# ArseneAmoya/image-retrieval-wavelet

Measured on AMD Instinct MI355X. Metric: query images/sec + mAP@5000, MIRFLICKR-25k 64-bit hash, 1/2/4/8 MI355X, higher is better.
Workload: dtype f32; 1 GPU; c1: MIRFLICKR-25k shape, retrieval-only: per GPU per step 2048 query images 3x224x224 u8 -> SWT db2 L3 -> band-attention head (Nq=4, E=384; DINOv2 backbone out of scope, CLS features synthetic) -> 64-bit hash -> Hamming top-5000 vs 25,000 codes -> mAP@5000; queries_per_gpu=2048, db_codes=25000, nbits=64, k=5000, wavelet=db2, level=3, arithmetic=fp32 SWT and head (fp32 MFMA), 64-bit popcount ranking, AP in fp32/fp64, streams=1, clock_steps=40, backend=none, parallelism=single GPU

## Files before the change

image-retrieval-wavelet_amd/csrc/ap_walk.hpp:

```cpp
#pragma once
#include "common.hpp"

namespace wv {

constexpr int kApRounds = 32;

template <int TPQ>
__host__ __device__ constexpr int ap_scratch_dwords() { return kApRounds * (TPQ / 64) + 2 * (TPQ / 64) + 2; }

struct ApState {
    uint32_t running = 0;
    double acc = 0.0;
};

template <int TPQ>
__device__ __forceinline__ void ap_accum(uint32_t relbits, const uint32_t *cnt, int Rc, int r_base, int t, ApState &st)
{
    constexpr int NW = TPQ / 64, CH = 8;
    const int wv = t >> 6;
    for (int r0 = 0; r0 < Rc; r0 += CH) {
        uint32_t c[CH][NW];
#pragma unroll
        for (int u = 0; u < CH; ++u)
#pragma unroll
            for (int w2 = 0; w2 < NW; ++w2) c[u][w2] = cnt[min(r0 + u, Rc - 1) * NW + w2];
#pragma unroll
        for (int u = 0; u < CH; ++u) {
            const int r = r0 + u;
            if (r < Rc) {
                uint32_t before = st.running, tot = 0;
#pragma unroll
                for (int w2 = 0; w2 < NW; ++w2) {
                    before += w2 < wv ? c[u][w2] : 0u;
                    tot += c[u][w2];
                }
                const bool rel = (relbits >> r) & 1u;
                const uint64_t m = __ballot(rel);
                if (rel) {
                    const uint32_t j = before + (uint32_t)mbcnt(m) + 1;
                    st.acc += (double)((float)j / (float)((r_base + r) * TPQ + t + 1));
                }
                st.running += tot;
            }
        }
    }
}

template <int TPQ, typename SYNC>
__device__ __forceinline__ void ap_final(const ApState &st, double *wsum, int t, float *__restrict__ ap_out,
                                         int32_t *__restrict__ nrel_out, SYNC group_barrier)
{
    constexpr int NW = TPQ / 64;
    const int lane = t & 63, wv = t >> 6;
    const double acc = wave_sum_f64(st.acc);
    if (lane == 0) wsum[wv] = acc;
    group_barrier();
    if (t == 0) {
        double s = wsum[0];
#pragma unroll
        for (int w2 = 1; w2 < NW; ++w2) s += wsum[w2];
        *ap_out = st.running ? (float)(s / (double)st.running) : 0.0f;
        if (nrel_out) *nrel_out = (int32_t)st.running;
    }
}

constexpr int kMaxCutoffs = 16;

struct ApCuts {
    int n;
    int k[kMaxCutoffs];
};

template <int TPQ>
__host__ __device__ constexpr int ap_cuts_scratch_dwords() { return ap_scratch_dwords<TPQ>() + TPQ / 64; }

template <int TPQ, typename SYNC>
__device__ __forceinline__ void ap_accum_cuts(uint32_t relbits, const uint32_t *cnt, int Rc, int r_base, int t, ApState &st,
                                              const ApCuts &cuts, int &next, double *wsum, uint32_t *wcut,
                                              float *__restrict__ ap_out, int32_t *__restrict__ nrel_out, SYNC group_barrier)
{
    constexpr int NW = TPQ / 64, CH = 8;
    const int lane = t & 63, wv = t >> 6;
    int64_t cut = next < cuts.n ? cuts.k[next] : INT64_MAX;
    for (int r0 = 0; r0 < Rc; r0 += CH) {
        uint32_t c[CH][NW];
#pragma unroll
        for (int u = 0; u < CH; ++u)
#pragma unroll
            for (int w2 = 0; w2 < NW; ++w2) c[u][w2] = cnt[min(r0 + u, Rc - 1) * NW + w2];
#pragma unroll
        for (int u = 0; u < CH; ++u) {
            const int r = r0 + u;
            if (r < Rc) {
                uint32_t before = st.running, tot = 0;
#pragma unroll
                for (int w2 = 0; w2 < NW; ++w2) {
                    before += w2 < wv ? c[u][w2] : 0u;
                    tot += c[u][w2];
                }
                const bool rel = (relbits >> r) & 1u;
                const uint64_t m = __ballot(rel);
                const int p = (r_base + r) * TPQ + t;
                double own = 0.0;
                if (rel) {
                    const uint32_t j = before + (uint32_t)mbcnt(m) + 1;
                    own = (double)((float)j / (float)(p + 1));
                }
                while (cut <= (int64_t)(r_base + r + 1) * TPQ) {
                    const bool in = rel && p < cut;
                    const uint64_t mc = __ballot(in);
                    const double acc = wave_sum_f64(in ? st.acc + own : st.acc);
                    if (lane == 0) {
                        wsum[wv] = acc;
                        wcut[wv] = (uint32_t)__popcll(mc);
                    }
                    group_barrier();
                    if (t == 0) {
                        double s = wsum[0];
                        uint32_t running = st.running + wcut[0];
#pragma unroll
                        for (int w2 = 1; w2 < NW; ++w2) {
                            s += wsum[w2];
                            running += wcut[w2];
                        }
                        ap_out[next] = running ? (float)(s / (double)running) : 0.0f;
                        if (nrel_out) nrel_out[next] = (int32_t)running;
                    }
                    group_barrier();
                    ++next;
                    cut = next < cuts.n ? cuts.k[next] : INT64_MAX;
                }
                if (rel) st.acc += own;
                st.running += tot;
            }
        }
    }
}

}
```

image-retrieval-wavelet_amd/csrc/rank.hpp:

```cpp
#pragma once
#include "common.hpp"

namespace wv {

struct ApCuts;

constexpr int kTopkThreads = 256;
constexpr int kMaxBins = 130;
constexpr int kWinBins = 32;
constexpr int kWinRows = kWinBins + 1;
constexpr size_t kRankLdsLimit = 100 * 1024;

enum class RankKernel {
    none,
    column,
    window256,
    window64,
};

enum class RankMode {
    lists,
    rows16,
    hist,
    ap,
    relbits,
    radius,
};

constexpr int64_t kImg64MaxRows = 64 * 64;
constexpr int64_t kImg256MaxRows = 256 * 128;

constexpr int rank_threads_per_query(RankKernel kern) { return kern == RankKernel::window64 ? 64 : 256; }

struct RankPlan {
    RankKernel kernel;
    int C;
    int NC;
    size_t lds;
    const char *why;
    const char *instead;
};

__host__ __device__ inline int rank2_bitmap_words(int64_t N) { return (int)((N + 31) / 32); }

inline size_t window_lds_bytes_per_query(int tpq, int k, int bm_words = 0)
{
    size_t b = (size_t)kWinRows * (tpq / 2) * 4;
    b += ((size_t)(k + tpq) * 2 + 15) / 16 * 16;
    b += (size_t)(kMaxBins + 1 + kWinBins + 4 + 3) / 4 * 4 * 4;
    b += (size_t)bm_words * 4;
    b = (b + 15) / 16 * 16;
    const size_t hist = (size_t)(kMaxBins + 1) * 17 * 4;
    return b > hist ? b : (hist + 15) / 16 * 16;
}

constexpr int rank_radius_bitmap_words(int C) { return 8 * C + 1; }
inline size_t radius_lds_bytes(int C)
{
    const size_t b = (size_t)(kMaxBins + 1) * 16 * 4 + (size_t)2 * (kMaxBins + 1) * 4 + (size_t)rank_radius_bitmap_words(C) * 4;
    return (b + 15) / 16 * 16;
}

inline bool column_u16(int64_t n_items) { return n_items < 65536; }
inline size_t column_lds_bytes(int nbins, bool u16)
{
    const size_t h = (size_t)nbins * (u16 ? kTopkThreads / 2 : kTopkThreads);
    return (h + kMaxBins + kMaxBins + 1 + 4 + 3) / 4 * 4 * sizeof(uint32_t);
}

inline RankPlan rank_plan_column(int64_t N, int nbits)
{
    return {RankKernel::column, (int)ceil_div(N, kTopkThreads), 0, column_lds_bytes(nbits + 1, column_u16(N)), nullptr, ""};
}

inline RankKernel rank_window_kernel(int Q, int64_t N, int k)
{
    const char *force = ::wv::tune("WV_TOPK_V2");
    if (force && force[0] == '0') return RankKernel::none;
    if (N >= 65536 || 2 * (k + 128) >= 65536) return RankKernel::none;
    const bool fits256 = N <= kImg256MaxRows && window_lds_bytes_per_query(256, k) <= kRankLdsLimit;
    const bool fits64 = N <= kImg64MaxRows && 4 * window_lds_bytes_per_query(64, k) <= kRankLdsLimit;
    if (force && atoi(force) == 64 && fits64) return RankKernel::window64;
    if (force && atoi(force) == 256 && fits256) return RankKernel::window256;
    if (fits64 && Q >= 4096) return RankKernel::window64;
    return fits256 ? RankKernel::window256 : (fits64 ? RankKernel::window64 : RankKernel::none);
}

inline RankPlan rank_plan(int Q, int64_t N, int nbits, int k, RankMode mode)
{
    const bool fused = mode == RankMode::ap || mode == RankMode::relbits;
    const char *instead = mode == RankMode::ap ? "; call wv_hamming_topk + wv_map_at_k instead" : "";
    RankKernel kern = rank_window_kernel(Q, N, std::max(k, 1));
    if (kern == RankKernel::none) {
        if (mode == RankMode::lists) return rank_plan_column(N, nbits);
        return {RankKernel::none, 0, 0, 0, "are outside the windowed kernel (rows <= 32768, 16-bit row numbers: 2 (k + 128) < 65536)",
                instead};
    }
    if (fused && kern == RankKernel::window64 && k > 32 * 64) kern = RankKernel::window256;
    if (mode == RankMode::radius) kern = RankKernel::window256;
    RankPlan p{kern, 0, 0, 0, nullptr, ""};
    const int tpq = rank_threads_per_query(kern);
    p.C = (int)ceil_div(N, tpq);
    p.NC = p.C <= 16 ? 4 : (p.C <= 32 ? 8 : (p.C <= 64 ? 16 : (p.C <= 100 ? 25 : 32)));
    p.lds = window_lds_bytes_per_query(tpq, k, fused ? rank2_bitmap_words(N) : 0) * (kTopkThreads / tpq);
    if (mode == RankMode::radius) p.lds = radius_lds_bytes(p.C);
    if (fused && p.lds > kRankLdsLimit)
        return {RankKernel::none, 0, 0, 0, "do not fit the fused kernel's LDS (list + relevance bitmap)", instead};
    return p;
}

inline int rank_refuse(const char *what, const RankPlan &p, int64_t N, int k)
{
    WV_FAIL(WV_ENOTSUP, "%s: %lld rows / k=%d %s%s", what, (long long)N, k, p.why, p.instead);
}

inline size_t rank_image_bytes(RankKernel kern, int64_t N, int words)
{
    if (kern == RankKernel::column) return (size_t)ceil_div(N, kTopkThreads) * kTopkThreads * words * sizeof(uint64_t);
    const int tpq = rank_threads_per_query(kern);
    const int64_t C = ceil_div(N, tpq), rows = words == 1 ? (C + 1) / 2 : C;
    return (size_t)rows * tpq * 16;
}

struct BlobLayout {
    size_t column, window256, window64, total;
};
inline BlobLayout blob_layout(int64_t N, int words)
{
    BlobLayout L;
    L.column = L.window256 = L.window64 = L.total = (size_t)align_up((int64_t)dist_prepared_bytes(N, words), 256);
    if (words > 2) return L;
    L.window256 = L.column + (size_t)align_up((int64_t)rank_image_bytes(RankKernel::column, N, words), 256);
    L.window64 = L.window256 + (N <= kImg256MaxRows ? (size_t)align_up((int64_t)rank_image_bytes(RankKernel::window256, N, words), 256) : 0);
    L.total = L.window64 + (N <= kImg64MaxRows ? rank_image_bytes(RankKernel::window64, N, words) : 0);
    return L;
}
inline const void *blob_image(const void *prepared, int64_t N, int words, RankKernel kern)
{
    const BlobLayout L = blob_layout(N, words);
    return (const char *)prepared + (kern == RankKernel::column ? L.column : (kern == RankKernel::window256 ? L.window256 : L.window64));
}

int rank2_prepare(const uint64_t *db, void *img, int64_t N, int words, RankKernel kern, hipStream_t st);
size_t rank2_labels_bytes(int64_t N, int lwords);
int rank2_labels_prepare(const uint64_t *dblab, void *cls, int64_t N, int lwords, hipStream_t st);

struct Rank2Ap {
    const uint32_t *cls;
    const uint64_t *qlab;
    int lwords;
    float *ap;
    int32_t *nrel;
    uint64_t *relbits;
    int64_t relbits_ld;
    int64_t cum_ld;
};

int rank2_launch(const RankPlan &plan, const uint64_t *q, const void *img, int32_t *idx, uint16_t *rows16, uint8_t *dist,
                 uint32_t *cum, int Q, int64_t N, int nbits, int k, int64_t idx_offset, hipStream_t st,
                 const Rank2Ap *apx = nullptr, const ApCuts *cuts = nullptr);

int rank2_radius_launch(const RankPlan &plan, const uint64_t *q, const void *img, const Rank2Ap &apx, uint32_t *cum, uint32_t *cumrel,
                        int Q, int64_t N, int nbits, hipStream_t st);

}
```

image-retrieval-wavelet_amd/csrc/rank2.hip:

```cpp
#include "rank.hpp"
#include "ap_walk.hpp"

namespace wv {

#ifdef WV_RANK2_STAMPS
__device__ unsigned long long g_rank2_stamps[8];
#define R2_STAMP(i) do { __builtin_amdgcn_sched_barrier(0); const unsigned long long now_ = __builtin_amdgcn_s_memtime(); \
    __builtin_amdgcn_s_waitcnt(0xC07F); if (t == 0) atomicAdd(&g_rank2_stamps[i], now_ - stamp_); stamp_ = __builtin_amdgcn_s_memtime(); \
    __builtin_amdgcn_sched_barrier(0); } while (0)
#define R2_STAMP_INIT unsigned long long stamp_ = __builtin_amdgcn_s_memtime()
#else
#define R2_STAMP(i) do { } while (0)
#define R2_STAMP_INIT do { } while (0)
#endif

template <int WORDS>
struct QCode {
    uint64_t w[WORDS];
};

template <int TPQ>
__device__ __forceinline__ void group_sync()
{
    if constexpr (TPQ == 64) {
// ... 552 lines not shown

template <int WORDS, int TPQ, int NC, bool AP>
__global__ __launch_bounds__(256, rank2_min_waves(NC)) void k_rank_window(const uint64_t *__restrict__ q, const uint4 *__restrict__ img,
                                                     int32_t *__restrict__ idx, uint16_t *__restrict__ rows16,
                                                     uint8_t *__restrict__ dist, int Q, int64_t N, int C, int nbins, int k,
                                                     int64_t idx_offset, uint32_t *__restrict__ cum, int lds_per_group, Rank2Ap apx)
{
    extern __shared__ uint4 lds4[];
    constexpr int GPW = 256 / TPQ;
    const int g = threadIdx.x / TPQ, t = threadIdx.x % TPQ;
    const int qi = blockIdx.x * GPW + g;
    if (qi >= Q) return;
    uint8_t *lds = reinterpret_cast<uint8_t *>(lds4) + (size_t)g * lds_per_group;
    QCode<WORDS> qc;
#pragma unroll
    for (int w = 0; w < WORDS; ++w) {
        const uint64_t v = q[(int64_t)qi * WORDS + w];
        qc.w[w] = ((uint64_t)(uint32_t)__builtin_amdgcn_readfirstlane((int)(uint32_t)(v >> 32)) << 32) |
                  (uint32_t)__builtin_amdgcn_readfirstlane((int)(uint32_t)v);
    }
    if (k != 0) rank2_zero_table<TPQ>(lds, t);
    uint32_t dc[NC], dmin;
    rank2_distances<WORDS, TPQ, NC>(img, qc, N, C, t, dc, dmin);
#pragma unroll
    for (int once = 0; once < 1; ++once) {
        if (k == 0) {
            rank2_hist_only<TPQ, NC>(dc, N, C, nbins, cum + (int64_t)qi * (nbins + 1), lds, t);
            continue;
        }
        group_sync<TPQ>();
        if constexpr (AP) {
            const uint64_t lw = apx.qlab[(int64_t)qi * apx.lwords], lw2 = apx.lwords > 1 ? apx.qlab[(int64_t)qi * apx.lwords + 1] : 0;
            const uint64_t ql = ((uint64_t)(uint32_t)__builtin_amdgcn_readfirstlane((int)(uint32_t)(lw >> 32)) << 32) |
                                (uint32_t)__builtin_amdgcn_readfirstlane((int)(uint32_t)lw);
            const uint64_t ql2 = ((uint64_t)(uint32_t)__builtin_amdgcn_readfirstlane((int)(uint32_t)(lw2 >> 32)) << 32) |
                                 (uint32_t)__builtin_amdgcn_readfirstlane((int)(uint32_t)lw2);
            rank2_rank<TPQ, NC, 1>(dc, dmin, N, C, nbins, k,
                                      cum ? cum + (int64_t)qi * (apx.cum_ld ? apx.cum_ld : nbins + 1) : nullptr, nullptr, lds, t,
                                      apx.cls, ql, ql2, apx.ap ? apx.ap + qi : nullptr, apx.nrel ? apx.nrel + qi : nullptr,
                                      apx.relbits ? apx.relbits + (int64_t)qi * (apx.relbits_ld ? apx.relbits_ld : (k + 63) / 64)
                                                  : nullptr);
        } else {
            rank2_rank<TPQ, NC>(dc, dmin, N, C, nbins, k, cum ? cum + (int64_t)qi * (nbins + 1) : nullptr,
                                dist ? dist + (int64_t)qi * k : nullptr, lds, t);
            rank2_copy_list<TPQ>(lds, k, idx_offset, idx ? idx + (int64_t)qi * k : nullptr,
                                 rows16 ? rows16 + (int64_t)qi * k : nullptr, t);
        }
    }
}

constexpr int rank2_cuts_min_waves(int nc) { return nc <= 8 ? 6 : rank2_min_waves(nc); }

template <int WORDS, int TPQ, int NC>
__global__ __launch_bounds__(256, rank2_cuts_min_waves(NC)) void k_rank_window_cuts(const uint64_t *__restrict__ q, const uint4 *__restrict__ img,
                                                                               int Q, int64_t N, int C, int nbins, int lds_per_group,
                                                                               Rank2Ap apx, ApCuts cuts)
{
    extern __shared__ uint4 lds4[];
    constexpr int GPW = 256 / TPQ;
    const int g = threadIdx.x / TPQ, t = threadIdx.x % TPQ;
    const int qi = blockIdx.x * GPW + g;
    if (qi >= Q) return;
    uint8_t *lds = reinterpret_cast<uint8_t *>(lds4) + (size_t)g * lds_per_group;
    QCode<WORDS> qc;
#pragma unroll
    for (int w = 0; w < WORDS; ++w) {
        const uint64_t v = q[(int64_t)qi * WORDS + w];
        qc.w[w] = ((uint64_t)(uint32_t)__builtin_amdgcn_readfirstlane((int)(uint32_t)(v >> 32)) << 32) |
                  (uint32_t)__builtin_amdgcn_readfirstlane((int)(uint32_t)v);
    }
    rank2_zero_table<TPQ>(lds, t);
    uint32_t dc[NC], dmin;
    rank2_distances<WORDS, TPQ, NC>(img, qc, N, C, t, dc, dmin);
    group_sync<TPQ>();
    const uint64_t lw = apx.qlab[(int64_t)qi * apx.lwords], lw2 = apx.lwords > 1 ? apx.qlab[(int64_t)qi * apx.lwords + 1] : 0;
    const uint64_t ql = ((uint64_t)(uint32_t)__builtin_amdgcn_readfirstlane((int)(uint32_t)(lw >> 32)) << 32) |
                        (uint32_t)__builtin_amdgcn_readfirstlane((int)(uint32_t)lw);
    const uint64_t ql2 = ((uint64_t)(uint32_t)__builtin_amdgcn_readfirstlane((int)(uint32_t)(lw2 >> 32)) << 32) |
                         (uint32_t)__builtin_amdgcn_readfirstlane((int)(uint32_t)lw2);
    rank2_rank<TPQ, NC, 2>(dc, dmin, N, C, nbins, cuts.k[cuts.n - 1], nullptr, nullptr, lds, t, apx.cls, ql, ql2,
                           apx.ap + (int64_t)qi * cuts.n, apx.nrel ? apx.nrel + (int64_t)qi * cuts.n : nullptr, nullptr, &cuts);
}

template <int TPQ, int NC>
__device__ __forceinline__ void rank2_radius_hist(const uint32_t (&dc)[NC], int C, int nbins, const uint32_t *bitmap, uint32_t *table,
                                                  uint32_t *tot, uint32_t *__restrict__ cum_out, uint32_t *__restrict__ cumrel_out, int t)
{
    const int first = t * C;
    char *cell = reinterpret_cast<char *>(table) + (uint32_t)(t & 15) * 4u;
#pragma unroll
    for (int bw = 0; bw < NC; bw += 8) {
        if (bw * 4 < C) {
            const int p = first + bw * 4;
            const uint32_t lo = bitmap[p >> 5], hi = bitmap[(p >> 5) + 1];
            const uint32_t rel32 = (uint32_t)((((uint64_t)hi << 32) | lo) >> (p & 31));
#pragma unroll
            for (int j = 0; j < 32; ++j) {
                if (bw + (j >> 2) < NC) {
                    const uint32_t d = (dc[bw + (j >> 2)] >> (8 * (j & 3))) & 0xffu;
                    const uint32_t b = min(d, (uint32_t)nbins);
                    const uint32_t inc = 1u + (((rel32 >> j) & 1u) << 16);
                    __hip_atomic_fetch_add(reinterpret_cast<uint32_t *>(cell + b * 64), inc, __ATOMIC_RELAXED,
                                           __HIP_MEMORY_SCOPE_WORKGROUP);
                }
            }
            __builtin_amdgcn_sched_barrier(0);
        }
    }
    group_sync<TPQ>();
    for (int b = t; b < nbins; b += TPQ) {
        const uint4 *row = reinterpret_cast<const uint4 *>(table + b * 16);
        uint32_t all = 0, rel = 0;
#pragma unroll
        for (int i = 0; i < 4; ++i) {
            const uint4 v = row[i];
            all += (v.x & 0xffffu) + (v.y & 0xffffu) + (v.z & 0xffffu) + (v.w & 0xffffu);
            rel += (v.x >> 16) + (v.y >> 16) + (v.z >> 16) + (v.w >> 16);
        }
        tot[b] = all;
        tot[kMaxBins + 1 + b] = rel;
    }
    group_sync<TPQ>();
    if (t < 128) {
        const int which = __builtin_amdgcn_readfirstlane(t >> 6), b0 = 3 * (t & 63);
        const uint32_t *src = tot + which * (kMaxBins + 1);
        uint32_t *dst = which ? cumrel_out : cum_out;
        const uint32_t t0 = b0 < nbins ? src[b0] : 0u, t1 = b0 + 1 < nbins ? src[b0 + 1] : 0u, t2 = b0 + 2 < nbins ? src[b0 + 2] : 0u;
        const uint32_t incl = wave_incl_scan_u32(t0 + t1 + t2), excl = incl - (t0 + t1 + t2);
        if (b0 <= nbins) dst[b0] = excl;
        if (b0 + 1 <= nbins) dst[b0 + 1] = excl + t0;
        if (b0 + 2 <= nbins) dst[b0 + 2] = excl + t0 + t1;
    }
}

template <int WORDS, int TPQ, int NC>
__global__ __launch_bounds__(256, rank2_min_waves(NC)) void k_rank_radius(const uint64_t *__restrict__ q, const uint4 *__restrict__ img,
                                                                          int Q, int64_t N, int C, int nbins, Rank2Ap apx,
                                                                          uint32_t *__restrict__ cum, uint32_t *__restrict__ cumrel)
{
    static_assert(TPQ == 256, "the radius histograms are built for 256 threads per query (rank_plan never picks another)");
    extern __shared__ uint4 lds4[];
    const int t = threadIdx.x;
    const int qi = blockIdx.x;
    if (qi >= Q) return;
    uint32_t *table = reinterpret_cast<uint32_t *>(lds4);
    uint32_t *tot = table + (kMaxBins + 1) * 16;
    uint32_t *bitmap = tot + 2 * (kMaxBins + 1);
    QCode<WORDS> qc;
#pragma unroll
    for (int w = 0; w < WORDS; ++w) {
        const uint64_t v = q[(int64_t)qi * WORDS + w];
        qc.w[w] = ((uint64_t)(uint32_t)__builtin_amdgcn_readfirstlane((int)(uint32_t)(v >> 32)) << 32) |
                  (uint32_t)__builtin_amdgcn_readfirstlane((int)(uint32_t)v);
    }
    const int nw = rank2_bitmap_words(N);
    for (int i = t; i < (nbins + 1) * 16; i += TPQ) table[i] = 0;
    for (int w = nw + t; w < rank_radius_bitmap_words(C); w += TPQ) bitmap[w] = 0;
    uint32_t dc[NC], dmin;
    rank2_distances<WORDS, TPQ, NC>(img, qc, N, C, t, dc, dmin);
    (void)dmin;
    const uint64_t lw = apx.qlab[(int64_t)qi * apx.lwords], lw2 = apx.lwords > 1 ? apx.qlab[(int64_t)qi * apx.lwords + 1] : 0;
    const uint64_t ql = ((uint64_t)(uint32_t)__builtin_amdgcn_readfirstlane((int)(uint32_t)(lw >> 32)) << 32) |
                        (uint32_t)__builtin_amdgcn_readfirstlane((int)(uint32_t)lw);
    const uint64_t ql2 = ((uint64_t)(uint32_t)__builtin_amdgcn_readfirstlane((int)(uint32_t)(lw2 >> 32)) << 32) |
                         (uint32_t)__builtin_amdgcn_readfirstlane((int)(uint32_t)lw2);
    rank2_relevance_bitmap<TPQ>(apx.cls, ql, ql2, nw, t, bitmap);
    group_sync<TPQ>();
    rank2_radius_hist<TPQ, NC>(dc, C, nbins, bitmap, table, tot, cum + (int64_t)qi * (nbins + 1), cumrel + (int64_t)qi * (nbins + 1), t);
}

int rank2_prepare(const uint64_t *db, void *img, int64_t N, int words, RankKernel kern, hipStream_t st)
{
    const int tpq = rank_threads_per_query(kern);
    const int C = (int)ceil_div(N, tpq);
    const int64_t total = (int64_t)(words == 1 ? (C + 1) / 2 : C) * tpq;
    const unsigned grid = (unsigned)std::min<int64_t>(ceil_div(total, 256), 4096);
    if (words == 1)
        hipLaunchKernelGGL((k_rank2_image<1>), dim3(grid), dim3(256), 0, st, db, (uint4 *)img, N, C, tpq);
    else
        hipLaunchKernelGGL((k_rank2_image<2>), dim3(grid), dim3(256), 0, st, db, (uint4 *)img, N, C, tpq);
    WV_CHECK_LAUNCH("k_rank2_image");
    return WV_OK;
}

namespace {
struct WindowArgs {
    const uint64_t *q;
    const void *img;
    int32_t *idx;
    uint16_t *rows16;
    uint8_t *dist;
    uint32_t *cum;
    int Q;
    int64_t N;
    int nbins, k;
    int64_t idx_offset;
    hipStream_t st;
    bool fused;
    Rank2Ap apx;
    const ApCuts *cuts;
};

template <int WORDS, int TPQ, int NC>
int launch_window(const RankPlan &plan, const WindowArgs &a)
{
    constexpr int GPW = 256 / TPQ;
    if (a.cuts) {
        auto kc = k_rank_window_cuts<WORDS, TPQ, NC>;
        if (plan.lds > 64 * 1024) {
            hipError_t e = hipFuncSetAttribute(reinterpret_cast<const void *>(kc), hipFuncAttributeMaxDynamicSharedMemorySize, (int)plan.lds);
            if (e != hipSuccess) WV_FAIL(WV_EHIP, "rank_window_cuts: hipFuncSetAttribute(%zu): %s", plan.lds, hipGetErrorString(e));
        }
        hipLaunchKernelGGL(kc, dim3((unsigned)ceil_div(a.Q, GPW)), dim3(256), plan.lds, a.st, a.q, (const uint4 *)a.img, a.Q, a.N, plan.C,
                           a.nbins, (int)(plan.lds / GPW), a.apx, *a.cuts);
        WV_CHECK_LAUNCH("k_rank_window_cuts");
        return WV_OK;
    }
    auto kern = a.fused ? k_rank_window<WORDS, TPQ, NC, true> : k_rank_window<WORDS, TPQ, NC, false>;
    if (plan.lds > 64 * 1024) {
        hipError_t e = hipFuncSetAttribute(reinterpret_cast<const void *>(kern), hipFuncAttributeMaxDynamicSharedMemorySize, (int)plan.lds);
        if (e != hipSuccess) WV_FAIL(WV_EHIP, "rank_window: hipFuncSetAttribute(%zu): %s", plan.lds, hipGetErrorString(e));
    }
    hipLaunchKernelGGL(kern, dim3((unsigned)ceil_div(a.Q, GPW)), dim3(256), plan.lds, a.st, a.q, (const uint4 *)a.img, a.idx, a.rows16,
                       a.dist, a.Q, a.N, plan.C, a.nbins, a.k, a.idx_offset, a.cum, (int)(plan.lds / GPW), a.apx);
    WV_CHECK_LAUNCH("k_rank_window");
    return WV_OK;
}

template <int WORDS, int TPQ>
int launch_window_nc(const RankPlan &plan, const WindowArgs &a)
{
    if (plan.NC == 4) return launch_window<WORDS, TPQ, 4>(plan, a);
    if (plan.NC == 8) return launch_window<WORDS, TPQ, 8>(plan, a);
    if constexpr (TPQ == 256) {
        if (plan.NC == 25) return launch_window<WORDS, TPQ, 25>(plan, a);
        if (plan.NC == 32) return launch_window<WORDS, TPQ, 32>(plan, a);
    }
    return launch_window<WORDS, TPQ, 16>(plan, a);
}
}

int rank2_launch(const RankPlan &plan, const uint64_t *q, const void *img, int32_t *idx, uint16_t *rows16, uint8_t *dist,
                 uint32_t *cum, int Q, int64_t N, int nbits, int k, int64_t idx_offset, hipStream_t st, const Rank2Ap *apx,
                 const ApCuts *cuts)
{
    const WindowArgs a{q, img, idx, rows16, dist, cum, Q, N, nbits + 1, k, idx_offset, st, apx != nullptr, apx ? *apx : Rank2Ap{}, cuts};
    const bool wave = plan.kernel == RankKernel::window64;
    if (nbits <= 64) return wave ? launch_window_nc<1, 64>(plan, a) : launch_window_nc<1, 256>(plan, a);
    return wave ? launch_window_nc<2, 64>(plan, a) : launch_window_nc<2, 256>(plan, a);
}

namespace {
template <int WORDS, int NC>
int launch_radius(const RankPlan &plan, const uint64_t *q, const void *img, const Rank2Ap &apx, uint32_t *cum, uint32_t *cumrel, int Q,
                  int64_t N, int nbins, hipStream_t st)
{
    hipLaunchKernelGGL((k_rank_radius<WORDS, 256, NC>), dim3((unsigned)Q), dim3(256), plan.lds, st, q, (const uint4 *)img, Q, N, plan.C,
                       nbins, apx, cum, cumrel);
    WV_CHECK_LAUNCH("k_rank_radius");
    return WV_OK;
}

template <int WORDS>
int launch_radius_nc(const RankPlan &plan, const uint64_t *q, const void *img, const Rank2Ap &apx, uint32_t *cum, uint32_t *cumrel, int Q,
                     int64_t N, int nbins, hipStream_t st)
{
    if (plan.NC == 4) return launch_radius<WORDS, 4>(plan, q, img, apx, cum, cumrel, Q, N, nbins, st);
    if (plan.NC == 8) return launch_radius<WORDS, 8>(plan, q, img, apx, cum, cumrel, Q, N, nbins, st);
    if (plan.NC == 16) return launch_radius<WORDS, 16>(plan, q, img, apx, cum, cumrel, Q, N, nbins, st);
    if (plan.NC == 25) return launch_radius<WORDS, 25>(plan, q, img, apx, cum, cumrel, Q, N, nbins, st);
    return launch_radius<WORDS, 32>(plan, q, img, apx, cum, cumrel, Q, N, nbins, st);
}
}

int rank2_radius_launch(const RankPlan &plan, const uint64_t *q, const void *img, const Rank2Ap &apx, uint32_t *cum, uint32_t *cumrel,
                        int Q, int64_t N, int nbits, hipStream_t st)
{
    if (plan.kernel != RankKernel::window256) WV_FAIL(WV_EINVAL, "rank2_radius_launch: the plan names no 256-thread kernel");
    if (nbits <= 64) return launch_radius_nc<1>(plan, q, img, apx, cum, cumrel, Q, N, nbits + 1, st);
    return launch_radius_nc<2>(plan, q, img, apx, cum, cumrel, Q, N, nbits + 1, st);
}

}

#ifdef WV_RANK2_STAMPS
extern "C" int wv_debug_rank2_stamps(unsigned long long *host8)
{
    if (hipMemcpyFromSymbol(host8, HIP_SYMBOL(wv::g_rank2_stamps), 8 * sizeof(unsigned long long)) != hipSuccess) return -5;
    unsigned long long zero[8] = {0, 0, 0, 0, 0, 0, 0, 0};
    if (hipMemcpyToSymbol(HIP_SYMBOL(wv::g_rank2_stamps), zero, sizeof(zero)) != hipSuccess) return -5;
    return 0;
}
#endif
```

image-retrieval-wavelet_amd/csrc/topk.hip:

```cpp
#include "rank.hpp"
#include "ap_walk.hpp"

namespace wv {

template <int WORDS>
struct CodeSource {
    const uint64_t *dbT;
    uint64_t qw[WORDS];
    int64_t idx_offset;
    struct Raw {
        uint64_t w[WORDS];
    };
    __device__ __forceinline__ Raw fetch(int r, int t, int64_t) const
    {
        const uint64_t *p = dbT + ((int64_t)r * kTopkThreads + t) * WORDS;
        Raw c;
        if constexpr (WORDS == 2) {
            const uint4 v = *reinterpret_cast<const uint4 *>(p);
            c.w[0] = (uint64_t)v.x | ((uint64_t)v.y << 32);
            c.w[1] = (uint64_t)v.z | ((uint64_t)v.w << 32);
        } else {
#pragma unroll
            for (int w = 0; w < WORDS; ++w) c.w[w] = p[w];
        }
// ... 992 lines not shown
        if (int rc = require_workspace(what, workspace, workspace_bytes, Q, N, nbits, k)) return rc;
    hipStream_t st = (hipStream_t)stream;
    const void *img = nullptr;
    if (int rc = rank_image(plan, db, prepared, workspace, N, (nbits + 63) / 64, st, &img)) return rc;
    return rank2_launch(plan, q, img, nullptr, rows16, nullptr, cum, Q, N, nbits, k, 0, st);
}

extern "C" int wv_hamming_hist(const uint64_t *q, const uint64_t *db, const void *prepared, uint32_t *cum, int Q, int64_t N,
                               int nbits, void *workspace, size_t workspace_bytes, void *stream)
{
    if (int rc = validate_rank_shape("hamming_hist", q && cum && (db || prepared), Q, N, nbits)) return rc;
    if (Q == 0) return WV_OK;
    return shard_call("hamming_hist", RankMode::hist, q, db, prepared, nullptr, cum, Q, N, nbits, 0, workspace, workspace_bytes, stream);
}

extern "C" int wv_hamming_shard_prefix(const uint64_t *q, const uint64_t *db, const void *prepared, uint16_t *rows, uint32_t *cum,
                                       int Q, int64_t N, int nbits, int k, void *workspace, size_t workspace_bytes, void *stream)
{
    if (int rc = validate_rank_args("hamming_shard_prefix", q && rows && cum && (db || prepared), Q, N, nbits, k)) return rc;
    if (Q == 0) return WV_OK;
    return shard_call("hamming_shard_prefix", RankMode::rows16, q, db, prepared, rows, cum, Q, N, nbits, k, workspace, workspace_bytes,
                      stream);
}

extern "C" int wv_hamming_shard_relbits(const uint64_t *q, const void *prepared, const void *prepared_labels, const uint64_t *qlab,
                                        int lwords, uint64_t *relbits, int64_t relbits_ld, uint32_t *cum, int64_t cum_ld, int Q,
                                        int64_t N, int nbits, int k, void *stream)
{
    WV_REQUIRE(lwords >= 1, "hamming_shard_relbits: lwords=%d", lwords);
    if (lwords > 2) WV_FAIL(WV_ENOTSUP, "hamming_shard_relbits: %d label words (more than 128 classes)", lwords);
    WV_REQUIRE((relbits_ld == 0 || relbits_ld >= (k + 63) / 64) && (cum_ld == 0 || cum_ld >= nbits + 2),
               "hamming_shard_relbits: row pitches %lld / %lld too small", (long long)relbits_ld, (long long)cum_ld);
    if (int rc = validate_rank_args("hamming_shard_relbits", q && prepared && prepared_labels && qlab && relbits && cum, Q, N, nbits, k))
        return rc;
    if (Q == 0) return WV_OK;
    const Rank2Ap apx{(const uint32_t *)prepared_labels, qlab, lwords, nullptr, nullptr, relbits, relbits_ld, cum_ld};
    return fused_call("hamming_shard_relbits", RankMode::relbits, q, prepared, apx, cum, Q, N, nbits, k, stream);
}

extern "C" int wv_merge_relbits_map(const uint64_t *relbits, int64_t relbits_ld, const uint32_t *cum, int64_t cum_ld, int G, int Q,
                                    int kin, int k, int nbits, float *ap, int32_t *nrel, int32_t *need_out, void *stream)
{
    WV_REQUIRE((relbits_ld == 0 || relbits_ld >= (kin + 63) / 64) && (cum_ld == 0 || cum_ld >= nbits + 2),
               "merge_relbits_map: row pitches %lld / %lld too small", (long long)relbits_ld, (long long)cum_ld);
    WV_REQUIRE(relbits && cum && ap, "merge_relbits_map: null buffer");
    WV_REQUIRE(G >= 1 && Q >= 0 && kin >= 1 && k >= 1, "merge_relbits_map: bad shape G=%d Q=%d kin=%d k=%d", G, Q, kin, k);
    if (int rc = require_nbits("merge_relbits_map", nbits)) return rc;
    if (Q == 0) return WV_OK;
    const int nbins = nbits + 1, w32 = 2 * (int)ceil_div(kin, 64), mwords = (k + 31) / 32 + 1;
    const size_t lds = ((size_t)G * (nbins + 1) + nbins + 1 + mwords + (mwords & 1) + ap_scratch_dwords<256>() + 4) * 4;
    WV_REQUIRE(lds <= 60 * 1024, "merge_relbits_map: too many shards (G=%d)", G);
    hipLaunchKernelGGL(k_merge_relbits_ap, dim3(Q), dim3(256), lds, (hipStream_t)stream, reinterpret_cast<const uint32_t *>(relbits),
                       cum, G, Q, kin, w32, k, nbins, ap, nrel, need_out, relbits_ld ? 2 * relbits_ld : (int64_t)w32,
                       cum_ld ? cum_ld : (int64_t)(nbins + 1));
    WV_CHECK_LAUNCH("k_merge_relbits_ap");
    return WV_OK;
}

static int validate_cuts(const char *what, const int *ks, int nk, int64_t limit, const char *limit_name, ApCuts &cuts)
{
    static_assert(kMaxCutoffs == WV_MAX_CUTOFFS, "ap_walk.hpp and wvhash.h disagree");
    WV_REQUIRE(ks, "%s: null cut-off list", what);
    WV_REQUIRE(nk >= 1 && nk <= kMaxCutoffs, "%s: %d cut-offs (supported: 1..%d)", what, nk, kMaxCutoffs);
    cuts.n = nk;
    for (int i = 0; i < kMaxCutoffs; ++i) cuts.k[i] = i < nk ? ks[i] : 0;
    WV_REQUIRE(ks[0] >= 1, "%s: cut-off %d must be >= 1", what, ks[0]);
    for (int i = 1; i < nk; ++i)
        WV_REQUIRE(ks[i] > ks[i - 1], "%s: cut-offs must be strictly ascending (ks[%d]=%d after %d)", what, i, ks[i], ks[i - 1]);
    WV_REQUIRE(ks[nk - 1] <= limit, "%s: largest cut-off %d must be <= %s=%lld", what, ks[nk - 1], limit_name, (long long)limit);
    return WV_OK;
}

extern "C" int wv_hamming_map_at_ks(const uint64_t *q, const void *prepared, const void *prepared_labels, const uint64_t *qlab,
                                    int lwords, int Q, int64_t N, int nbits, const int *ks, int nk, float *ap, int32_t *nrel,
                                    void *stream)
{
    WV_REQUIRE(lwords >= 1, "hamming_map_at_ks: lwords=%d", lwords);
    if (lwords > 2) WV_FAIL(WV_ENOTSUP, "hamming_map_at_ks: %d label words (more than 128 classes): wv_hamming_topk + wv_map_at_ks", lwords);
    if (int rc = validate_rank_shape("hamming_map_at_ks", q && prepared && prepared_labels && qlab && ap, Q, N, nbits)) return rc;
    ApCuts cuts;
    if (int rc = validate_cuts("hamming_map_at_ks", ks, nk, N, "N", cuts)) return rc;
    if (Q == 0) return WV_OK;
    const int kmax = cuts.k[nk - 1];
    const RankPlan plan = rank_plan(Q, N, nbits, kmax, RankMode::ap);
    if (plan.kernel == RankKernel::none)
        WV_FAIL(WV_ENOTSUP, "hamming_map_at_ks: %lld rows / largest cut-off %d %s; call wv_hamming_topk + wv_map_at_ks instead",
                (long long)N, kmax, plan.why);
    const Rank2Ap apx{(const uint32_t *)prepared_labels, qlab, lwords, ap, nrel, nullptr, 0, 0};
    return rank2_launch(plan, q, blob_image(prepared, N, (nbits + 63) / 64, plan.kernel), nullptr, nullptr, nullptr, nullptr, Q, N, nbits,
                        kmax, 0, (hipStream_t)stream, &apx, &cuts);
}

extern "C" size_t wv_merge_relbits_map_ks_lds_bytes(int G, int kmax, int nbits)
{
    if (G < 1 || kmax < 1 || nbits < 1 || nbits > 128) return 0;
    const int nbins = nbits + 1;
    const size_t mwords = (size_t)(kmax + 31) / 32 + 1;
    return ((size_t)G * (nbins + 1) + nbins + 1 + ap_cuts_scratch_dwords<256>() + 4) * 4 + (mwords + (mwords & 1)) * 4;
}

extern "C" int wv_merge_relbits_map_ks(const uint64_t *relbits, int64_t relbits_ld, const uint32_t *cum, int64_t cum_ld, int G, int Q,
                                       int kin, const int *ks, int nk, int nbits, float *ap, int32_t *nrel, int32_t *need_out,
                                       void *stream)
{
    WV_REQUIRE((relbits_ld == 0 || relbits_ld >= (kin + 63) / 64) && (cum_ld == 0 || cum_ld >= nbits + 2),
               "merge_relbits_map_ks: row pitches %lld / %lld too small", (long long)relbits_ld, (long long)cum_ld);
    WV_REQUIRE(relbits && cum && ap, "merge_relbits_map_ks: null buffer");
    WV_REQUIRE(G >= 1 && Q >= 0 && kin >= 1, "merge_relbits_map_ks: bad shape G=%d Q=%d kin=%d", G, Q, kin);
    if (int rc = require_nbits("merge_relbits_map_ks", nbits)) return rc;
    ApCuts cuts;
    if (int rc = validate_cuts("merge_relbits_map_ks", ks, nk, 0x7fffffff, "INT_MAX", cuts)) return rc;
    if (Q == 0) return WV_OK;
    const int kmax = cuts.k[nk - 1], nbins = nbits + 1, w32 = 2 * (int)ceil_div(kin, 64);
    const size_t lds = wv_merge_relbits_map_ks_lds_bytes(G, kmax, nbits), limit = WV_MERGE_RELBITS_LDS_LIMIT;
    if (lds > limit)
        WV_FAIL(WV_ENOTSUP, "merge_relbits_map_ks: the merged string of the largest cut-off %d does not fit LDS beside the run boundaries "
                "of G=%d shards (%zu bytes needed, %zu available)", kmax, G, lds, limit);
    hipLaunchKernelGGL(k_merge_relbits_ap_cuts, dim3(Q), dim3(256), lds, (hipStream_t)stream, reinterpret_cast<const uint32_t *>(relbits),
                       cum, G, Q, kin, w32, nbins, ap, nrel, need_out, relbits_ld ? 2 * relbits_ld : (int64_t)w32,
                       cum_ld ? cum_ld : (int64_t)(nbins + 1), cuts);
    WV_CHECK_LAUNCH("k_merge_relbits_ap_cuts");
    return WV_OK;
}

extern "C" int wv_map_at_ks(const int32_t *idx, int64_t ld, int Q, const int *ks, int nk, const uint64_t *qlab, const uint64_t *dblab,
                            int lwords, float *ap, int32_t *nrel, void *stream)
{
    WV_REQUIRE(idx && qlab && dblab && ap, "map_at_ks: null buffer");
    WV_REQUIRE(Q >= 0 && lwords >= 1 && ld >= 1, "map_at_ks: bad shape Q=%d ld=%lld lwords=%d", Q, (long long)ld, lwords);
    ApCuts cuts;
    if (int rc = validate_cuts("map_at_ks", ks, nk, ld, "ld", cuts)) return rc;
    if (Q == 0) return WV_OK;
    hipStream_t st = (hipStream_t)stream;
    if (lwords == 1)
        hipLaunchKernelGGL((k_map_at_ks<1>), dim3(Q), dim3(256), 0, st, idx, ld, qlab, dblab, lwords, ap, nrel, cuts);
    else if (lwords == 2)
        hipLaunchKernelGGL((k_map_at_ks<2>), dim3(Q), dim3(256), 0, st, idx, ld, qlab, dblab, lwords, ap, nrel, cuts);
    else
        hipLaunchKernelGGL((k_map_at_ks<0>), dim3(Q), dim3(256), 0, st, idx, ld, qlab, dblab, lwords, ap, nrel, cuts);
    WV_CHECK_LAUNCH("k_map_at_ks");
    return WV_OK;
}

extern "C" int wv_hamming_topk_rows16(const uint64_t *q, const uint64_t *db, const void *prepared, uint16_t *rows, int Q,
                                      int64_t N, int nbits, int k, void *workspace, size_t workspace_bytes, void *stream)
{
    if (int rc = validate_rank_args("hamming_topk_rows16", q && rows && (db || prepared), Q, N, nbits, k)) return rc;
    if (Q == 0) return WV_OK;
    return shard_call("hamming_topk_rows16", RankMode::rows16, q, db, prepared, rows, nullptr, Q, N, nbits, k, workspace, workspace_bytes,
                      stream);
}
```

Before: 1.612 million query images/s.

## Add order-free fused AP kernel using per-bin atomic ranks with relevance counts

Adds a new fused rank+mAP kernel for the single-cutoff AP mode. It places each item with LDS atomics that pack a position count and a relevant count into one word, so every relevant item gets its rank and its precision term directly. This replaces the ordered list build and sequential walk. Per-thread relevance bits are computed from the class bitmaps in registers instead of a shared relevance bitmap. The planner selects the kernel when 3k >= N, N <= 32767 and k fits, and keeps the old window path for the multi-cutoff entry point. The cost is more LDS atomic traffic and a second placement pass per bin window.

```diff
diff --git a/image-retrieval-wavelet_amd/csrc/ap_walk.hpp b/image-retrieval-wavelet_amd/csrc/ap_walk.hpp
--- a/image-retrieval-wavelet_amd/csrc/ap_walk.hpp
+++ b/image-retrieval-wavelet_amd/csrc/ap_walk.hpp
@@ -46,21 +46,50 @@
     }
 }
 
+template <int TPQ>
+__device__ __forceinline__ void ap_wave_sums(double thread_acc, double *wsum, int t)
+{
+    const double acc = wave_sum_f64(thread_acc);
+    if ((t & 63) == 0) wsum[t >> 6] = acc;
+}
+template <int TPQ>
+__device__ __forceinline__ void ap_store(const double *wsum, uint32_t running, float *__restrict__ ap_out, int32_t *__restrict__ nrel_out)
+{
+    constexpr int NW = TPQ / 64;
+    double s = wsum[0];
+#pragma unroll
+    for (int w2 = 1; w2 < NW; ++w2) s += wsum[w2];
+    *ap_out = running ? (float)(s / (double)running) : 0.0f;
+    if (nrel_out) *nrel_out = (int32_t)running;
+}
+
 template <int TPQ, typename SYNC>
 __device__ __forceinline__ void ap_final(const ApState &st, double *wsum, int t, float *__restrict__ ap_out,
                                          int32_t *__restrict__ nrel_out, SYNC group_barrier)
 {
+    ap_wave_sums<TPQ>(st.acc, wsum, t);
+    group_barrier();
+    if (t == 0) ap_store<TPQ>(wsum, st.running, ap_out, nrel_out);
+}
+
+constexpr int kApOrderFreeMaxK = 1 << 15;
+
+__device__ __forceinline__ void ap_add_rank(uint32_t j, uint32_t p, double &acc) { acc += (double)((float)j / (float)(p + 1)); }
+
+template <int TPQ, typename SYNC>
+__device__ __forceinline__ void ap_final_ranks(double thread_acc, uint32_t hits, double *wsum, uint32_t *whits, int t,
+                                               float *__restrict__ ap_out, int32_t *__restrict__ nrel_out, SYNC group_barrier)
+{
     constexpr int NW = TPQ / 64;
-    const int lane = t & 63, wv = t >> 6;
-    const double acc = wave_sum_f64(st.acc);
-    if (lane == 0) wsum[wv] = acc;
+    ap_wave_sums<TPQ>(thread_acc, wsum, t);
+    const uint32_t wave_hits = wave_sum_u32(hits);
+    if ((t & 63) == 0) whits[t >> 6] = wave_hits;
     group_barrier();
     if (t == 0) {
-        double s = wsum[0];
+        uint32_t running = 0;
 #pragma unroll
-        for (int w2 = 1; w2 < NW; ++w2) s += wsum[w2];
-        *ap_out = st.running ? (float)(s / (double)st.running) : 0.0f;
-        if (nrel_out) *nrel_out = (int32_t)st.running;
+        for (int w2 = 0; w2 < NW; ++w2) running += whits[w2];
+        ap_store<TPQ>(wsum, running, ap_out, nrel_out);
     }
 }
 
diff --git a/image-retrieval-wavelet_amd/csrc/rank.hpp b/image-retrieval-wavelet_amd/csrc/rank.hpp
--- a/image-retrieval-wavelet_amd/csrc/rank.hpp
+++ b/image-retrieval-wavelet_amd/csrc/rank.hpp
@@ -10,6 +10,9 @@
 constexpr int kWinBins = 32;
 constexpr int kWinRows = kWinBins + 1;
 constexpr size_t kRankLdsLimit = 100 * 1024;
+constexpr int64_t kApRanksMaxRows = 32767;
+constexpr int kApRanksMaxK = 32639;
+constexpr int ap_ranks_win_bins(int nbits) { return nbits + 1 <= 24 ? 24 : 32; }
 
 enum class RankKernel {
     none,
@@ -37,6 +40,7 @@
     int C;
     int NC;
     size_t lds;
+    int ap_win_bins;
     const char *why;
     const char *instead;
 };
@@ -54,6 +58,8 @@
     return b > hist ? b : (hist + 15) / 16 * 16;
 }
 
+inline size_t ap_ranks_lds_bytes(int win_bins) { return (size_t)(win_bins + 1) * 256 * 4 + 32 * 4 + 8 * 4 + 4 * 8; }
+
 constexpr int rank_radius_bitmap_words(int C) { return 8 * C + 1; }
 inline size_t radius_lds_bytes(int C)
 {
@@ -70,7 +76,7 @@
 
 inline RankPlan rank_plan_column(int64_t N, int nbits)
 {
-    return {RankKernel::column, (int)ceil_div(N, kTopkThreads), 0, column_lds_bytes(nbits + 1, column_u16(N)), nullptr, ""};
+    return {RankKernel::column, (int)ceil_div(N, kTopkThreads), 0, column_lds_bytes(nbits + 1, column_u16(N)), 0, nullptr, ""};
 }
 
 inline RankKernel rank_window_kernel(int Q, int64_t N, int k)
@@ -86,26 +92,33 @@
     return fits256 ? RankKernel::window256 : (fits64 ? RankKernel::window64 : RankKernel::none);
 }
 
-inline RankPlan rank_plan(int Q, int64_t N, int nbits, int k, RankMode mode)
+inline RankPlan rank_plan(int Q, int64_t N, int nbits, int k, RankMode mode, bool single_cut = true)
 {
     const bool fused = mode == RankMode::ap || mode == RankMode::relbits;
     const char *instead = mode == RankMode::ap ? "; call wv_hamming_topk + wv_map_at_k instead" : "";
     RankKernel kern = rank_window_kernel(Q, N, std::max(k, 1));
     if (kern == RankKernel::none) {
         if (mode == RankMode::lists) return rank_plan_column(N, nbits);
-        return {RankKernel::none, 0, 0, 0, "are outside the windowed kernel (rows <= 32768, 16-bit row numbers: 2 (k + 128) < 65536)",
+        return {RankKernel::none, 0, 0, 0, 0, "are outside the windowed kernel (rows <= 32768, 16-bit row numbers: 2 (k + 128) < 65536)",
                 instead};
     }
     if (fused && kern == RankKernel::window64 && k > 32 * 64) kern = RankKernel::window256;
     if (mode == RankMode::radius) kern = RankKernel::window256;
-    RankPlan p{kern, 0, 0, 0, nullptr, ""};
+    RankPlan p{kern, 0, 0, 0, 0, nullptr, ""};
     const int tpq = rank_threads_per_query(kern);
     p.C = (int)ceil_div(N, tpq);
     p.NC = p.C <= 16 ? 4 : (p.C <= 32 ? 8 : (p.C <= 64 ? 16 : (p.C <= 100 ? 25 : 32)));
     p.lds = window_lds_bytes_per_query(tpq, k, fused ? rank2_bitmap_words(N) : 0) * (kTopkThreads / tpq);
     if (mode == RankMode::radius) p.lds = radius_lds_bytes(p.C);
     if (fused && p.lds > kRankLdsLimit)
-        return {RankKernel::none, 0, 0, 0, "do not fit the fused kernel's LDS (list + relevance bitmap)", instead};
+        return {RankKernel::none, 0, 0, 0, 0, "do not fit the fused kernel's LDS (list + relevance bitmap)", instead};
+    if (mode == RankMode::ap && single_cut && kern == RankKernel::window256 && N <= kApRanksMaxRows && k <= kApRanksMaxK) {
+        const char *pin = ::wv::tune("WV_RANK_AP");
+        const int pinned = pin ? atoi(pin) : 0;
+        if (pinned == 24 || pinned == 32) p.ap_win_bins = pinned;
+        else if (!(pin && pin[0] == 'w') && 3 * (int64_t)k >= N) p.ap_win_bins = ap_ranks_win_bins(nbits);
+        if (p.ap_win_bins) p.lds = ap_ranks_lds_bytes(p.ap_win_bins);
+    }
     return p;
 }
 
diff --git a/image-retrieval-wavelet_amd/csrc/rank2.hip b/image-retrieval-wavelet_amd/csrc/rank2.hip
--- a/image-retrieval-wavelet_amd/csrc/rank2.hip
+++ b/image-retrieval-wavelet_amd/csrc/rank2.hip
@@ -658,6 +658,189 @@
                            apx.ap + (int64_t)qi * cuts.n, apx.nrel ? apx.nrel + (int64_t)qi * cuts.n : nullptr, nullptr, &cuts);
 }
 
+
+template <int NC>
+constexpr int rank2_rel_words() { return (4 * NC + 31) / 32; }
+
+template <int NC>
+__device__ __forceinline__ void rank2_own_relevance(const uint32_t *__restrict__ cls, uint64_t ql, uint64_t ql_hi, int nw, int first,
+                                                    uint32_t (&rel)[rank2_rel_words<NC>()])
+{
+    constexpr int RW = rank2_rel_words<NC>();
+    uint32_t acc[RW + 1];
+    int wi[RW + 1];
+#pragma unroll
+    for (int i = 0; i <= RW; ++i) {
+        acc[i] = 0;
+        wi[i] = min((first >> 5) + i, nw - 1);
+    }
+    uint64_t m = ql;
+    int cbase = 0;
+    if (!m) { m = ql_hi; ql_hi = 0; cbase = 64; }
+    while (m) {
+        const int c0 = cbase + __builtin_ctzll(m);
+        m &= m - 1;
+        const int c1 = m ? cbase + __builtin_ctzll(m) : c0;
+        m &= m - 1;
+        const int c2 = m ? cbase + __builtin_ctzll(m) : c0;
+        m &= m - 1;
+        const int c3 = m ? cbase + __builtin_ctzll(m) : c0;
+        m &= m - 1;
+        uint32_t v[4][RW + 1];
+#pragma unroll
+        for (int i = 0; i <= RW; ++i) {
+            v[0][i] = cls[(size_t)c0 * nw + wi[i]];
+            v[1][i] = cls[(size_t)c1 * nw + wi[i]];
+            v[2][i] = cls[(size_t)c2 * nw + wi[i]];
+            v[3][i] = cls[(size_t)c3 * nw + wi[i]];
+        }
+#pragma unroll
+        for (int i = 0; i <= RW; ++i) acc[i] |= (v[0][i] | v[1][i]) | (v[2][i] | v[3][i]);
+        if (!m && ql_hi) { m = ql_hi; ql_hi = 0; cbase = 64; }
+    }
+#pragma unroll
+    for (int i = 0; i < RW; ++i) rel[i] = (uint32_t)((((uint64_t)acc[i + 1] << 32) | acc[i]) >> (first & 31));
+}
+
+template <int NC, int WB>
+__device__ __forceinline__ void rank2_rank_ap(const uint32_t (&dc)[NC], const uint32_t (&rel_in)[rank2_rel_words<NC>()], uint32_t dmin, int C,
+                                              int nbins, int k, uint8_t *lds_raw, int t, float *__restrict__ ap_out,
+                                              int32_t *__restrict__ nrel_out)
+{
+    static_assert(WB <= 32 && WB % 4 == 0, "one lane per bin in the scan of the totals, four waves share the bins");
+    static_assert(kApRanksMaxK <= kApOrderFreeMaxK && kApRanksMaxRows + 128 < 65536, "see ap_walk.hpp and the cell halves");
+    constexpr int TPQ = 256, NW = 4, ROWB = TPQ * 4;
+    uint32_t *table = reinterpret_cast<uint32_t *>(lds_raw);
+    uint32_t *tot = table + (WB + 1) * TPQ;
+    uint32_t *misc = tot + 32;
+    double *wsum = reinterpret_cast<double *>(misc + 8);
+    const int lane = t & 63, wv = __builtin_amdgcn_readfirstlane(t >> 6);
+    dmin = wave_min_u32(dmin);
+    if (lane == 0) misc[wv] = dmin;
+    __syncthreads();
+    dmin = (uint32_t)__builtin_amdgcn_readfirstlane((int)min(min(misc[0], misc[1]), min(misc[2], misc[3])));
+    int lo = min((int)dmin, nbins - 1);
+    uint32_t placed = 0;
+    char *col = reinterpret_cast<char *>(table) + (uint32_t)t * 4u;
+    double acc = 0.0;
+    uint32_t hits = 0;
+    uint32_t relv[rank2_rel_words<NC>()];
+#pragma unroll
+    for (int i = 0; i < rank2_rel_words<NC>(); ++i) relv[i] = rel_in[i];
+    for (;;) {
+#pragma unroll
+        for (int i = 0; i < rank2_rel_words<NC>(); ++i) asm volatile("" : "+v"(relv[i]));
+#pragma unroll
+        for (int bw = 0; bw < NC; bw += 2) {
+            if (bw * 4 < C) {
+#pragma unroll
+                for (int j = 0; j < 8; ++j) {
+                    if (bw + (j >> 2) < NC) {
+                        const int i = bw * 4 + j;
+                        const uint32_t d = (dc[bw + (j >> 2)] >> (8 * (j & 3))) & 0xffu;
+                        const uint32_t b = min(d - (uint32_t)lo, (uint32_t)WB);
+                        const uint32_t inc = 1u | (((relv[i >> 5] >> (i & 31)) & 1u) << 16);
+                        __hip_atomic_fetch_add(reinterpret_cast<uint32_t *>(col + b * ROWB), inc, __ATOMIC_RELAXED,
+                                               __HIP_MEMORY_SCOPE_WORKGROUP);
+                    }
+                }
+            }
+        }
+        __syncthreads();
+        for (int b = wv; b < WB; b += NW) {
+            const uint4 v = *reinterpret_cast<const uint4 *>(table + b * TPQ + 4 * lane);
+            const uint32_t s = wave_sum_u32(v.x + v.y + v.z + v.w);
+            if (lane == 0) tot[b] = s;
+        }
+        __syncthreads();
+        const uint32_t my_tot = lane < WB ? tot[lane] : 0u;
+        const uint32_t incl = wave_incl_scan_u32(my_tot);
+        const uint32_t bin_base = placed + incl - my_tot;
+        const uint32_t win_total = (uint32_t)__builtin_amdgcn_readlane((int)incl, 63);
+        for (int b = wv; b < WB; b += NW) {
+            const uint32_t base_b = (uint32_t)__builtin_amdgcn_readlane((int)bin_base, b);
+            uint4 *cell = reinterpret_cast<uint4 *>(table + b * TPQ + 4 * lane);
+            const uint4 v = *cell;
+            const uint32_t s4 = v.x + v.y + v.z + v.w;
+            const uint32_t e0 = wave_incl_scan_u32(s4) - s4 + base_b;
+            *cell = make_uint4(e0, e0 + v.x, e0 + v.x + v.y, e0 + v.x + v.y + v.z);
+        }
+        table[WB * TPQ + t] = (uint32_t)k;
+        __syncthreads();
+#pragma unroll
+        for (int i = 0; i < rank2_rel_words<NC>(); ++i) asm volatile("" : "+v"(relv[i]));
+        asm volatile("" : "+s"(lo));
+#pragma unroll
+        for (int bw = 0; bw < NC; bw += 4) {
+            if (bw * 4 < C) {
+                uint32_t old[16];
+#pragma unroll
+                for (int j = 0; j < 16; ++j) {
+                    old[j] = 0;
+                    if (bw + (j >> 2) < NC) {
+                        const int i = bw * 4 + j;
+                        const uint32_t d = (dc[bw + (j >> 2)] >> (8 * (j & 3))) & 0xffu;
+                        const uint32_t b = min(d - (uint32_t)lo, (uint32_t)WB);
+                        const uint32_t inc = 1u | (((relv[i >> 5] >> (i & 31)) & 1u) << 16);
+                        old[j] = __hip_atomic_fetch_add(reinterpret_cast<uint32_t *>(col + b * ROWB), inc, __ATOMIC_RELAXED,
+                                                        __HIP_MEMORY_SCOPE_WORKGROUP);
+                    }
+                }
+#pragma unroll
+                for (int j = 0; j < 16; ++j) {
+                    if (bw + (j >> 2) < NC) {
+                        const int i = bw * 4 + j;
+                        const uint32_t p = old[j] & 0xffffu;
+                        if (((relv[i >> 5] >> (i & 31)) & 1u) && p < (uint32_t)k) {
+                            ap_add_rank((old[j] >> 16) + 1u, p, acc);
+                            ++hits;
+                        }
+                    }
+                }
+                __builtin_amdgcn_sched_barrier(0);
+            }
+        }
+        placed += win_total;
+        lo += WB;
+        if (lo >= nbins || (placed & 0xffffu) >= (uint32_t)k) break;
+        __syncthreads();
+        for (int i = t; i < (WB + 1) * TPQ / 4; i += TPQ) reinterpret_cast<uint4 *>(table)[i] = make_uint4(0, 0, 0, 0);
+        __syncthreads();
+    }
+    ap_final_ranks<TPQ>(acc, hits, wsum, misc + 4, t, ap_out, nrel_out, [] { __syncthreads(); });
+}
+
+template <int WORDS, int NC, int WB>
+__global__ __launch_bounds__(256, rank2_min_waves(NC)) void k_rank_ap(const uint64_t *__restrict__ q, const uint4 *__restrict__ img, int Q,
+                                                                      int64_t N, int C, int nbins, int k, Rank2Ap apx)
+{
+    extern __shared__ uint4 lds4[];
+    constexpr int TPQ = 256;
+    const int t = threadIdx.x;
+    const int qi = blockIdx.x;
+    if (qi >= Q) return;
+    uint8_t *lds = reinterpret_cast<uint8_t *>(lds4);
+    QCode<WORDS> qc;
+#pragma unroll
+    for (int w = 0; w < WORDS; ++w) {
+        const uint64_t v = q[(int64_t)qi * WORDS + w];
+        qc.w[w] = ((uint64_t)(uint32_t)__builtin_amdgcn_readfirstlane((int)(uint32_t)(v >> 32)) << 32) |
+                  (uint32_t)__builtin_amdgcn_readfirstlane((int)(uint32_t)v);
+    }
+    const uint64_t lw = apx.qlab[(int64_t)qi * apx.lwords], lw2 = apx.lwords > 1 ? apx.qlab[(int64_t)qi * apx.lwords + 1] : 0;
+    const uint64_t ql = ((uint64_t)(uint32_t)__builtin_amdgcn_readfirstlane((int)(uint32_t)(lw >> 32)) << 32) |
+                        (uint32_t)__builtin_amdgcn_readfirstlane((int)(uint32_t)lw);
+    const uint64_t ql2 = ((uint64_t)(uint32_t)__builtin_amdgcn_readfirstlane((int)(uint32_t)(lw2 >> 32)) << 32) |
+                         (uint32_t)__builtin_amdgcn_readfirstlane((int)(uint32_t)lw2);
+    for (int i = t; i < (WB + 1) * TPQ / 4; i += TPQ) reinterpret_cast<uint4 *>(lds)[i] = make_uint4(0, 0, 0, 0);
+    uint32_t rel[rank2_rel_words<NC>()];
+    rank2_own_relevance<NC>(apx.cls, ql, ql2, rank2_bitmap_words(N), t * C, rel);
+    uint32_t dc[NC], dmin;
+    rank2_distances<WORDS, TPQ, NC>(img, qc, N, C, t, dc, dmin);
+    __syncthreads();
+    rank2_rank_ap<NC, WB>(dc, rel, dmin, C, nbins, k, lds, t, apx.ap + qi, apx.nrel ? apx.nrel + qi : nullptr);
+}
+
 template <int TPQ, int NC>
 __device__ __forceinline__ void rank2_radius_hist(const uint32_t (&dc)[NC], int C, int nbins, const uint32_t *bitmap, uint32_t *table,
                                                   uint32_t *tot, uint32_t *__restrict__ cum_out, uint32_t *__restrict__ cumrel_out, int t)
@@ -792,6 +975,17 @@
         WV_CHECK_LAUNCH("k_rank_window_cuts");
         return WV_OK;
     }
+    if constexpr (TPQ == 256) {
+        if (plan.ap_win_bins) {
+            WV_REQUIRE(a.fused && a.apx.ap && !a.apx.relbits && !a.cum && a.N <= kApRanksMaxRows && a.k <= kApRanksMaxK,
+                       "rank_ap: the plan does not match the call");
+            auto ka = plan.ap_win_bins == 32 ? k_rank_ap<WORDS, NC, 32> : k_rank_ap<WORDS, NC, 24>;
+            hipLaunchKernelGGL(ka, dim3((unsigned)a.Q), dim3(256), plan.lds, a.st, a.q, (const uint4 *)a.img, a.Q, a.N, plan.C, a.nbins,
+                               a.k, a.apx);
+            WV_CHECK_LAUNCH("k_rank_ap");
+            return WV_OK;
+        }
+    }
     auto kern = a.fused ? k_rank_window<WORDS, TPQ, NC, true> : k_rank_window<WORDS, TPQ, NC, false>;
     if (plan.lds > 64 * 1024) {
         hipError_t e = hipFuncSetAttribute(reinterpret_cast<const void *>(kern), hipFuncAttributeMaxDynamicSharedMemorySize, (int)plan.lds);
diff --git a/image-retrieval-wavelet_amd/csrc/topk.hip b/image-retrieval-wavelet_amd/csrc/topk.hip
--- a/image-retrieval-wavelet_amd/csrc/topk.hip
+++ b/image-retrieval-wavelet_amd/csrc/topk.hip
@@ -1098,7 +1098,7 @@
     if (int rc = validate_cuts("hamming_map_at_ks", ks, nk, N, "N", cuts)) return rc;
     if (Q == 0) return WV_OK;
     const int kmax = cuts.k[nk - 1];
-    const RankPlan plan = rank_plan(Q, N, nbits, kmax, RankMode::ap);
+    const RankPlan plan = rank_plan(Q, N, nbits, kmax, RankMode::ap, false);
     if (plan.kernel == RankKernel::none)
         WV_FAIL(WV_ENOTSUP, "hamming_map_at_ks: %lld rows / largest cut-off %d %s; call wv_hamming_topk + wv_map_at_ks instead",
                 (long long)N, kmax, plan.why);
```

Result: no change. 1.602 million query images/s (-0.6%).
